# OlegArenz/gmmvi

Measured on AMD Instinct MI355X. Metric: samples_components_per_sec, higher is better.
Workload: dtype f32; 1 GPU; ns: stm target D=20, K=100 components (100/GPU), 100 samples/component, N=10000 samples/iter, SAMTRON (Stein, fixed K, reuse ratio 0, KL trust regions, improvement-based stepsizes); K=100, D=20, N=10000, parallelism=component-shard x1

## Files before the change

gmmvi_amd/_lib.py:

```python
import ctypes as C
import os

_HERE = os.path.dirname(os.path.abspath(__file__))
LIB_PATH = os.environ.get("GMMVI_HIP_LIB", os.path.join(_HERE, "libgmmvi_hip.so"))

GAUSS, STUDENT_T = 0, 1
SELF_NORMALIZED, OWN_SAMPLES_ONLY, EXPLICIT_ESTIMATE = 1, 2, 4
MAX_DIM = 64
MORE_REGISTER_MAX_DIM = 21
MORE_BLOCKED_MIN_DIM, MORE_BLOCKED_MAX_DIM = 64, 128
MAX_DIM_BLOCKED = 512
MAX_DIM_DIAG = 131072
BLOCKED_ABOVE_DEFAULT = 50


_blocked_above = None


def _atoi(text):
    import re
    m = re.match(r"\s*([+-]?\d+)", text)
    return int(m.group(1)) if m else 0


# ... 67 lines not shown
    "gmmvi_target_bnn": (_i, [_p, _i, _i, _i, _i, _p, _p, _u64, _u32, _i, _f, _f, _p, _i, _p, _p]),
    "gmmvi_bnn_predict": (_i, [_p, _i, _i, _i, _p, _i, _p, _i, _p]),
    "gmmvi_target_talos": (_i, [_p, _p, _p, _p, _i, _p, _p]),
    "gmmvi_talos_fk": (_i, [_p, _p, _p, _i, _p, _p]),
    "gmmvi_sample_components": (_i, [_p, _i, _i, _p, _p, _p, _i, _u64, _u64, _i, _p, _p, _p]),
    "gmmvi_philox_normals": (_i, [_p, _u64, _u64, _i, _i, _i, _p]),
    "gmmvi_philox_uniforms": (_i, [_p, _u64, _u64, _i, _i, _p]),
    "gmmvi_stein": (_i, [_p, _i, _i, _p, _p, _i, _p, _p, _p, _p, _p, _i, _i, _p, _p]),
    "gmmvi_more": (_i, [_p, _i, _i, _p, _p, _p, _i, _p, _p, _p, _p, _p, _i, _i, _p, _p, _p]),
    "gmmvi_more_blocked": (_i, [_p, _i, _i, _p, _p, _p, _i, _p, _p, _p, _p, _p, _i, _i, _p, _p, _p]),
    "gmmvi_update_components_kl": (_i, [_p, _i, _i, _p, _p, _p, _p, _p, _f, _f, _p, _p, _p, _p, _p, _p, _p]),
    "gmmvi_update_components_kl_reference": (_i, [_p, _i, _i, _p, _p, _p, _p, _p, _f, _f, _p, _p, _p, _p, _p, _p]),
    "gmmvi_update_components_direct": (_i, [_p, _i, _i, _p, _p, _p, _p, _p, _f, _p, _p, _p]),
    "gmmvi_update_components_iblr": (_i, [_p, _i, _i, _p, _p, _p, _p, _p, _f, _p, _p, _p]),
    "gmmvi_expected_log_ratios": (_i, [_p, _i, _i, _p, _p, _p, _p, _f, _p, _i, _p, _p, _p]),
    "gmmvi_update_weights_kl": (_i, [_p, _i, _p, _p, _p, _f, _p]),
    "gmmvi_update_weights_direct": (_i, [_p, _i, _p, _p, _p, _f]),
    "gmmvi_component_stepsize_improvement": (_i, [_p, _i, _p, _p, _p, _f, _f, _f, _f]),
    "gmmvi_weight_stepsize_improvement": (_i, [_p, _i, _p, _p, _p, _f, _f, _f, _f]),
    "gmmvi_train_iter_samtron": (_i, [_p, _p]),
    "gmmvi_sharded_scratch_floats": (_sz, [_i, _i, _i]),
    "gmmvi_train_iter_sharded_phase": (_i, [_p, _p, _i]),
    "gmmvi_comm_unique_id": (_i, [C.c_char_p]),
    "gmmvi_comm_init": (_i, [_p, C.c_char_p, _i, _i]),
    "gmmvi_comm_destroy": (_i, [_p]),
    "gmmvi_allgather_f32": (_i, [_p, _p, _p, _sz]),
    "gmmvi_allreduce_f32": (_i, [_p, _p, _sz, _i]),
    "gmmvi_combine_partials": (_i, [_p, _i, _i, _i, _p, _p, _p, _p]),
    "gmmvi_diag_packed_stride": (_sz, [_i]),
    "gmmvi_diag_pack": (_i, [_p, _i, _i, _p, _p, _p]),
# ... 41 lines not shown
```

gmmvi_amd/csrc/api.hip:

```cpp
#include "common.h"
#include <cstring>
#include "blocked.h"

std::string g_gmmvi_global_err;

int gmmvi_ws_reserve(gmmvi_ctx* ctx, size_t nbytes) {
    ++ctx->ws_epoch;
    if (nbytes <= ctx->ws_bytes) return GMMVI_OK;
    GMMVI_HIP_CHECK(ctx, hipStreamSynchronize(ctx->stream));
    if (ctx->ws) GMMVI_HIP_CHECK(ctx, hipFree(ctx->ws));
    ctx->ws = nullptr;
    ctx->ws_bytes = 0;
    size_t want = nbytes + nbytes / 2;
    GMMVI_HIP_CHECK(ctx, hipMalloc(&ctx->ws, want));
    ctx->ws_bytes = want;
    return GMMVI_OK;
}

extern "C" {

int gmmvi_device_count(void) {
    int n = 0;
    if (hipGetDeviceCount(&n) != hipSuccess) return 0;
    return n;
// ... 6 lines not shown
    hipError_t e = hipGetDeviceCount(&n);
    if (e != hipSuccess || n == 0)
        return gmmvi_fail(nullptr, GMMVI_ERR_HIP, std::string("no HIP device: ") + hipGetErrorString(e));
    if (device < 0 || device >= n) return gmmvi_fail(nullptr, GMMVI_ERR_ARG, "device index out of range");
    gmmvi_ctx* ctx = new gmmvi_ctx();
    ctx->device = device;
    e = hipSetDevice(device);
    if (e == hipSuccess) e = hipStreamCreateWithFlags(&ctx->stream, hipStreamNonBlocking);
    if (e != hipSuccess) {
        g_gmmvi_global_err = std::string("gmmvi_ctx_create: ") + hipGetErrorString(e);
        delete ctx;
        return GMMVI_ERR_HIP;
    }
    hipDeviceProp_t prop;
    if (hipGetDeviceProperties(&prop, device) == hipSuccess) ctx->num_cus = prop.multiProcessorCount;
    *out = ctx;
    return GMMVI_OK;
}

void gmmvi_ctx_destroy(gmmvi_ctx* ctx) {
    if (!ctx) return;
    gmmvi_comm_destroy(ctx);
    if (ctx->stream) {
        (void)hipStreamSynchronize(ctx->stream);
        (void)hipStreamDestroy(ctx->stream);
    }
    if (ctx->ws) (void)hipFree(ctx->ws);
    if (ctx->arena) (void)hipFree(ctx->arena);
    if (ctx->bimg) (void)hipFree(ctx->bimg);
    if (ctx->up_ring) {
        for (int i = 0; i < gmmvi_ctx::UP_SLOTS; ++i) (void)hipEventDestroy(ctx->up_event[i]);
        (void)hipHostFree(ctx->up_ring);
    }
    if (ctx->defer_ws) (void)hipFree(ctx->defer_ws);
    delete ctx;
}

const char* gmmvi_last_error(gmmvi_ctx* ctx) { return ctx ? ctx->err.c_str() : g_gmmvi_global_err.c_str(); }

int gmmvi_sync(gmmvi_ctx* ctx) {
    GMMVI_HIP_CHECK(ctx, hipStreamSynchronize(ctx->stream));
    return GMMVI_OK;
}

int gmmvi_malloc(gmmvi_ctx* ctx, size_t nbytes, void** out_dev) {
    GMMVI_ARG_CHECK(ctx, out_dev != nullptr);
    *out_dev = nullptr;
    if (nbytes == 0) nbytes = 4;
    GMMVI_HIP_CHECK(ctx, hipSetDevice(ctx->device));
// ... 496 lines not shown
```

gmmvi_amd/csrc/common.h:

```cpp
#pragma once
#include <hip/hip_runtime.h>
#include <cstdio>
#include <cstring>
#include <cstdint>
#include <string>
#include <vector>
#include "../../include/gmmvi_hip.h"
#include "iter_prep.h"

struct CombineJob {
    int R = 0, N = 0, D = 0;
    long part_stride = 0;
    int first_block = 0, blocks = 0;
    const float* lp_parts = nullptr;
    const float* grad_parts = nullptr;
    const float* lp2_parts = nullptr;
    float* lp_out = nullptr;
    float* grad_out = nullptr;
    float* lp2_out = nullptr;
};

struct SampleJob {
    int K = 0, D = 0, uniform_count = 0;
    const float* means = nullptr; const float* chols = nullptr; const int32_t* offsets = nullptr;
// ... 23 lines not shown
    void* arena = nullptr;
    size_t arena_bytes = 0;
    static constexpr int UP_SLOTS = 64;
    static constexpr size_t UP_SLOT_BYTES = 64 * 1024;
    unsigned char* up_ring = nullptr;
    hipEvent_t up_event[UP_SLOTS] = {};
    bool up_used[UP_SLOTS] = {};
    int up_next = 0;
    void* bimg = nullptr;
    size_t bimg_bytes = 0;
    bool defer_combine = false;
    CombineJob pending;
    Riders riders;
    void* defer_ws = nullptr;
    size_t defer_bytes = 0;
    void* comm = nullptr;
    int n_ranks = 1, rank = 0;
    int num_cus = 256;
    unsigned func_attr_done = 0;
    bool prof = false;
    const char* prof_tag = nullptr;
    struct ProfRec { const char* name; hipEvent_t start, stop; double units; };
    std::vector<ProfRec> prof_recs;
};

struct GmmviProfScope {
    gmmvi_ctx* ctx; hipEvent_t stop = nullptr;
    GmmviProfScope(gmmvi_ctx* c, const char* name, double units = 0.0) : ctx(c) {
        if (!c->prof) return;
        hipEvent_t start;
// ... 48 lines not shown
CombineJob gmmvi_take_pending_combine(gmmvi_ctx* ctx, int threads, int first_block, bool light = false);
Riders gmmvi_take_pending_riders(gmmvi_ctx* ctx, int first_block, int threads, bool prep_only = false);
int gmmvi_flush_pending_riders(gmmvi_ctx* ctx);
struct SteinSlab;
int gmmvi_stein_partials(gmmvi_ctx* ctx, int K, int D, const float* packed_dev, const float* X_dev, int N, const float* ld_dev,
                         const float* qgrad_dev, const float* bg_dev, const float* tgrad_dev, int flags, SteinSlab* slab);
int gmmvi_stein_finalize_slab(gmmvi_ctx* ctx, int K, int D, const SteinSlab& slab, int N, int flags, const float* packed_dev,
                              float* H_neg_out_dev, float* g_neg_out_dev);
int gmmvi_update_components_kl_from_slab(gmmvi_ctx* ctx, int K, int D, const SteinSlab& slab, int N, int stein_flags,
                                         const float* packed_old_dev, float* H_neg_dev, float* g_neg_dev, float* means_dev,
                                         float* chols_dev, const float* stepsizes_dev, float temperature, float l2_init,
                                         float* last_eta_dev, float* l2_dev, float* num_received_updates_dev,
                                         int32_t* success_out_dev, float* packed_out_dev);
int gmmvi_update_weights_internal(gmmvi_ctx* ctx, int mode, int K, float* logw_dev, const float* E_dev,
                                  const float* stepsize_dev, float beta, float* kl_eta_out_dev, float* exp_out_dev);

inline int gmmvi_padded_dim(int D) {
    static const int dps[] = {2, 4, 8, 10, 12, 16, 20, 24, 32, 40, 50, 64};
    for (int dp : dps) if (D <= dp) return dp;
    return -1;
}

#define GMMVI_DISPATCH_DP(DPVAL, ...)                  \
    switch (DPVAL) {                                   \
        case 2:  { constexpr int DP = 2;  __VA_ARGS__; } break;  \
        case 4:  { constexpr int DP = 4;  __VA_ARGS__; } break;  \
        case 8:  { constexpr int DP = 8;  __VA_ARGS__; } break;  \
        case 10: { constexpr int DP = 10; __VA_ARGS__; } break;  \
        case 12: { constexpr int DP = 12; __VA_ARGS__; } break;  \
        case 16: { constexpr int DP = 16; __VA_ARGS__; } break;  \
// ... 103 lines not shown
```

gmmvi_amd/csrc/fused.hip:

```cpp
#include "common.h"
#include "stepsize_rules.h"
#include "iter_prep.h"
#include "stein_finalize.h"

namespace {
struct Arena {
    float *ld, *lq, *qgrad, *bg, *H, *g, *E;
    int32_t *mapping, *success;
};

}

static int arena_reserve(gmmvi_ctx* ctx, size_t floats) {
    if (floats * sizeof(float) <= ctx->arena_bytes) return GMMVI_OK;
    GMMVI_HIP_CHECK(ctx, hipStreamSynchronize(ctx->stream));
    if (ctx->arena) GMMVI_HIP_CHECK(ctx, hipFree(ctx->arena));
    ctx->arena = nullptr;
    ctx->arena_bytes = 0;
    size_t want = floats * sizeof(float) * 3 / 2;
    GMMVI_HIP_CHECK(ctx, hipMalloc(&ctx->arena, want));
    ctx->arena_bytes = want;
    return GMMVI_OK;
}

// ... 2 lines not shown
        int rc__ = (call);             \
        if (rc__ != GMMVI_OK) return rc__; \
    } while (0)

static int train_iter_samtron_body(gmmvi_ctx* ctx, const gmmvi_samtron_plan* p);

extern "C" int gmmvi_train_iter_samtron(gmmvi_ctx* ctx, const gmmvi_samtron_plan* p) {
    GMMVI_ARG_CHECK(ctx, ctx != nullptr);
    int rc = gmmvi_flush_pending_combine(ctx);
    if (rc == GMMVI_OK) rc = train_iter_samtron_body(ctx, p);
    if (rc != GMMVI_OK) {
        ctx->pending = CombineJob();
        ctx->riders.prep_blocks = ctx->riders.sample_blocks = 0;
        ctx->defer_combine = false;
        ctx->prof_tag = nullptr;
    }
    return rc;
}

static int train_iter_samtron_body(gmmvi_ctx* ctx, const gmmvi_samtron_plan* p) {
    GMMVI_ARG_CHECK(ctx, p != nullptr);
    GMMVI_ARG_CHECK(ctx, (p->target_kind >= 0 && p->target_kind <= 2) || p->target_kind == 4);
    GMMVI_ARG_CHECK(ctx, p->target_kind != 2 || (p->logreg_A && p->logreg_M >= 1 && p->logreg_prior_std > 0.f));
    GMMVI_ARG_CHECK(ctx, p->target_kind != 4 || (p->talos_model && p->talos_context && p->D == 34));
    const int K = p->K, D = p->D, N = p->N;
    GMMVI_ARG_CHECK(ctx, K >= 1 && D >= 1 && D < GMMVI_MAX_DIM && N >= 1);
    GMMVI_ARG_CHECK(ctx, p->means && p->chols && p->logw && p->packed && p->packed_new && p->stepsizes && p->last_eta &&
                             p->l2 && p->num_updates && p->offsets && p->bg_logw && p->db_samples && p->db_tlp &&
                             p->db_tgrad && p->db_mapping && p->reward_next && p->wstate);
    GMMVI_ARG_CHECK(ctx, p->n_old >= 0 && p->max_per_component >= 0 && p->phase >= 0 && p->phase <= 2);
// ... 103 lines not shown
    ctx->defer_combine = true;
    ctx->prof_tag = "sweep_post";
    int rc_post = gmmvi_mixture_eval(ctx, GMMVI_GAUSS, 0.f, K, D, p->packed_new, p->logw, xa, Na, a.ld, a.lq, nullptr);
    ctx->defer_combine = false;
    ctx->prof_tag = nullptr;
    GMMVI_TRY(rc_post);
    if (p->presample_next && n_old == 0) {
        const int max_pc = p->max_per_component > 0 ? p->max_per_component : (N + K - 1) / K;
        SampleJob& sj = ctx->riders.sample;
        sj.K = K; sj.D = D; sj.uniform_count = (long)K * max_pc == N ? max_pc : 0;
        sj.means = p->means; sj.chols = p->chols; sj.offsets = p->offsets;
        sj.seed = p->seed; sj.first_index = p->first_index + (uint64_t)N;
        sj.X = x + (size_t)N * D; sj.mapping = p->db_mapping + N; sj.mapping_base = p->mapping_base + K;
        ctx->riders.sample_blocks = K * ((max_pc + 255) / 256);
    }
    GMMVI_TRY(gmmvi_expected_log_ratios(ctx, K, Na, a.ld, a.bg, tlp_a, a.lq, p->temperature, p->logw,
                                        (p->stein_flags & GMMVI_SELF_NORMALIZED) ? 1 : 0, a.E, p->reward_next, nullptr));
    GMMVI_TRY(gmmvi_flush_pending_riders(ctx));
    if (K > 1) {
        GMMVI_TRY(gmmvi_update_weights_internal(ctx, p->weight_update_mode == 0 ? 0 : 1, K, p->logw, a.E, p->wstate,
                                                p->temperature, nullptr, p->weight_slot));
    }
    return GMMVI_OK;
}


namespace {
struct ShardArena { float *ld, *lq, *bg, *qgrad, *H, *g, *E; int32_t* success; };
}
extern "C" size_t gmmvi_sharded_scratch_floats(int K, int D, int N) {
    if (K < 1 || D < 1 || N < 1) return 0;
    return (size_t)K * N + 2 * (size_t)N + (size_t)N * D + (size_t)K * D * D + (size_t)K * D + 2 * (size_t)K + 64;
}
static void shard_arena(float* base, int K, int D, int N, ShardArena& a) {
    a.ld = base; base += (size_t)K * N;
    a.lq = base; base += N;
    a.bg = base; base += N;
// ... 141 lines not shown
```

gmmvi_amd/csrc/weights.hip:

```cpp
#include "common.h"
#include "riders.h"
#include "stepsize_rules.h"
#include "wave_reduce.h"
#include "combine.h"
#include <cfloat>

namespace {

__device__ __forceinline__ float wsum(float v) { return gmmvi_wave_sum(v); }
__device__ __forceinline__ float wmax(float v) { return gmmvi_wave_max(v); }

__device__ float block_max(float v, float* red) {
    v = wmax(v);
    __syncthreads();
    if ((threadIdx.x & 63) == 0) red[threadIdx.x >> 6] = v;
    __syncthreads();
    return fmaxf(fmaxf(red[0], red[1]), fmaxf(red[2], red[3]));
}
__device__ float block_sum(float v, float* red) {
    v = wsum(v);
    __syncthreads();
    if ((threadIdx.x & 63) == 0) red[threadIdx.x >> 6] = v;
    __syncthreads();
    return (red[0] + red[1]) + (red[2] + red[3]);
}

template <int R>
__device__ __forceinline__ void elr_accumulate(int N, const float* __restrict__ row, const float* __restrict__ bg,
                                               const float* __restrict__ tlp, const float* __restrict__ logq, int Rrt, float beta,
                                               float& m, float& s, float& se, float& s2) {
    constexpr int B = 4;
    for (int n0 = threadIdx.x; n0 < N; n0 += 1024 * B) {
        float av[B], rv[B];
#pragma unroll
        for (int u = 0; u < B; ++u) {
            const int n = min(n0 + 1024 * u, N - 1);
            av[u] = row[n] - bg[n];
            float lq;
            if constexpr (R == 0) lq = logq[n];
            else if constexpr (R > 0) lq = combine_log_values_n<R>(logq, N, n);
            else lq = combine_log_values(logq, Rrt, N, n);
            rv[u] = tlp[n] - beta * lq;
        }
#pragma unroll
        for (int u = 0; u < B; ++u) {
            if (n0 + 1024 * u < N) {
                const float a = av[u], rho = rv[u];
                const float mn = fmaxf(m, a);
                const float sc = __expf(m - mn), e = __expf(a - mn);
                s = fmaf(s, sc, e);
                se = fmaf(se, sc, e * rho);
                s2 = fmaf(s2, sc * sc, e * e);
                m = mn;
            }
        }
    }
}

__device__ __forceinline__ void elr_body(int N, const float* __restrict__ ld, const float* __restrict__ bg,
                                         const float* __restrict__ tlp, const float* __restrict__ logq, int logq_R,
                                         float beta, const float* __restrict__ logw, int self_normalized,
                                         float* __restrict__ E_out, float* __restrict__ reward_out,
                                         float* __restrict__ ess_out) {
    __shared__ float red[4][16];
    const int k = blockIdx.x;
    const float* row = ld + (size_t)k * N;
    float m = -3.0e38f, s = 0.f, se = 0.f, s2 = 0.f;
    switch (logq_R) {
        case 0: elr_accumulate<0>(N, row, bg, tlp, logq, 0, beta, m, s, se, s2); break;
        case 2: elr_accumulate<2>(N, row, bg, tlp, logq, 2, beta, m, s, se, s2); break;
        case 3: elr_accumulate<3>(N, row, bg, tlp, logq, 3, beta, m, s, se, s2); break;
        case 4: elr_accumulate<4>(N, row, bg, tlp, logq, 4, beta, m, s, se, s2); break;
        case 5: elr_accumulate<5>(N, row, bg, tlp, logq, 5, beta, m, s, se, s2); break;
        case 6: elr_accumulate<6>(N, row, bg, tlp, logq, 6, beta, m, s, se, s2); break;
        case 7: elr_accumulate<7>(N, row, bg, tlp, logq, 7, beta, m, s, se, s2); break;
        case 8: elr_accumulate<8>(N, row, bg, tlp, logq, 8, beta, m, s, se, s2); break;
        case 10: elr_accumulate<10>(N, row, bg, tlp, logq, 10, beta, m, s, se, s2); break;
        case 12: elr_accumulate<12>(N, row, bg, tlp, logq, 12, beta, m, s, se, s2); break;
        case 16: elr_accumulate<16>(N, row, bg, tlp, logq, 16, beta, m, s, se, s2); break;
        default: elr_accumulate<-1>(N, row, bg, tlp, logq, logq_R, beta, m, s, se, s2); break;
    }
    const float mw = wmax(m);
    const float f = __expf(m - mw);
    s = wsum(s * f); se = wsum(se * f); s2 = wsum(s2 * f * f);
    const int lane = threadIdx.x & 63, wave = threadIdx.x >> 6;
    if (lane == 0) { red[0][wave] = mw; red[1][wave] = s; red[2][wave] = se; red[3][wave] = s2; }
    __syncthreads();
    if (threadIdx.x == 0) {
        float M = -3.0e38f;
        for (int w = 0; w < 16; ++w) M = fmaxf(M, red[0][w]);
        float S = 0.f, SE = 0.f, S2 = 0.f;
        for (int w = 0; w < 16; ++w) {
            const float g = __expf(red[0][w] - M);
            S = fmaf(red[1][w], g, S); SE = fmaf(red[2][w], g, SE); S2 = fmaf(red[3][w], g * g, S2);
        }
        const float E = self_normalized ? SE / S : SE * __expf(M) / (float)N;
        if (E_out) E_out[k] = E;
        if (reward_out) reward_out[k] = beta * logw[k] + E;
        if (ess_out) ess_out[k] = (S * S) / S2;
    }
}

__global__ __launch_bounds__(1024) void elr_kernel(int N, const float* __restrict__ ld, const float* __restrict__ bg,
                                                   const float* __restrict__ tlp, const float* __restrict__ logq, int logq_R,
                                                   float beta, const float* __restrict__ logw, int self_normalized,
                                                   float* __restrict__ E_out, float* __restrict__ reward_out,
                                                   float* __restrict__ ess_out) {
    elr_body(N, ld, bg, tlp, logq, logq_R, beta, logw, self_normalized, E_out, reward_out, ess_out);
}

template <int DP>
__global__ __launch_bounds__(1024) void elr_riders_kernel(int N, const float* __restrict__ ld, const float* __restrict__ bg,
                                                          const float* __restrict__ tlp, const float* __restrict__ logq,
                                                          int logq_R, float beta, const float* __restrict__ logw,
                                                          int self_normalized, float* __restrict__ E_out,
                                                          float* __restrict__ reward_out, float* __restrict__ ess_out,
                                                          Riders riders) {
    extern __shared__ __align__(16) float sm_riders[];
    if (riders_carried<DP>(riders, sm_riders)) return;
    elr_body(N, ld, bg, tlp, logq, logq_R, beta, logw, self_normalized, E_out, reward_out, ess_out);
}

__device__ float wave_lse(const float* v, int K) {
    const int t = threadIdx.x;
    float m = -3.0e38f;
    for (int i = t; i < K; i += 64) m = fmaxf(m, v[i]);
    m = wmax(m);
    float s = 0.f;
    for (int i = t; i < K; i += 64) s += __expf(v[i] - m);
    s = wsum(s);
    return m + __logf(s);
}

__device__ float weights_kl(float eta, float beta, const float* lw, const float* E, float* nl, int K) {
    const int t = threadIdx.x;
// ... 73 lines not shown
    }
    if (lb == ub) {
    } else if (ub_ok) {
        eta = expf(ub);
        kl = weights_kl_reg<NE>(eta, beta, lw, E, h, v);
    } else {
        updated = false;
        kl = -1.f; eta = -1.f;
    }
#pragma unroll
    for (int e = 0; e < NE; ++e)
        if (h[e]) nl[t + 64 * e] = v[e];
    __syncthreads();
}

__global__ __launch_bounds__(64) void update_weights_kernel(int mode, int K, float* __restrict__ logw,
                                                            const float* __restrict__ E_in, const float* __restrict__ stepsize,
                                                            float beta, float* __restrict__ kl_eta_out,
                                                            float* __restrict__ exp_out) {
    extern __shared__ float sm[];
    float* lw = sm; float* E = sm + K; float* nl = sm + 2 * K;
    const int t = threadIdx.x;
    for (int i = t; i < K; i += 64) { lw[i] = logw[i]; E[i] = E_in[i]; nl[i] = logw[i]; }
    __syncthreads();
    if (K <= 1) return;
    const float bound = stepsize[0];
    float kl = -1.f, eta = -1.f;
    bool updated = true;
    if (mode == 1) {
        for (int i = t; i < K; i += 64) nl[i] = lw[i] + bound / beta * E[i];
        __syncthreads();
        float l = wave_lse(nl, K);
        for (int i = t; i < K; i += 64) nl[i] = fmaxf(nl[i] - l, -69.07f);
        __syncthreads();
        l = wave_lse(nl, K);
// ... 31 lines not shown
        }
    }
    if (!updated) {
        for (int i = t; i < K; i += 64) nl[i] = lw[i];
        __syncthreads();
    }
    const float l = wave_lse(nl, K);
    for (int i = t; i < K; i += 64) {
        const float v = nl[i] - l;
        logw[i] = v;
        if (exp_out) exp_out[i] = expf(v);
    }
    if (t == 0 && kl_eta_out) { kl_eta_out[0] = kl; kl_eta_out[1] = eta; }
}

__global__ void component_stepsize_kernel(int K, float* __restrict__ stepsizes, const float* __restrict__ prev,
                                          const float* __restrict__ last, float mn, float mx, float inc, float dec) {
    const int k = blockIdx.x * blockDim.x + threadIdx.x;
    if (k >= K) return;
    stepsizes[k] = component_stepsize_rule(stepsizes[k], prev[k], last[k], mn, mx, inc, dec);
}

__global__ __launch_bounds__(64) void weight_stepsize_kernel(int K, const float* __restrict__ logw,
                                                             const float* __restrict__ rewards_last, float* __restrict__ state,
                                                             float mn, float mx, float inc, float dec) {
    weight_stepsize_wave(K, logw, rewards_last, state, mn, mx, inc, dec, threadIdx.x);
}

}

extern "C" {

int gmmvi_expected_log_ratios(gmmvi_ctx* ctx, int K, int N, const float* ld_dev, const float* bg_dev,
                              const float* tlp_dev, const float* logq_dev, float beta, const float* logw_dev,
                              int self_normalized, float* E_out_dev, float* reward_out_dev, float* ess_out_dev) {
    GMMVI_ARG_CHECK(ctx, K >= 1 && N >= 1);
    GMMVI_ARG_CHECK(ctx, ld_dev && bg_dev && tlp_dev && logq_dev && logw_dev);
    int logq_R = 0;
    {
        const CombineJob& j = ctx->pending;
        if (j.R > 0 && j.lp_out == logq_dev && j.N == N && !j.grad_out && !j.lp2_out) {
            logq_R = j.R;
            logq_dev = j.lp_parts;
            ctx->pending = CombineJob();
        } else {
            int rc = gmmvi_flush_pending_combine(ctx);
            if (rc != GMMVI_OK) return rc;
        }
    }
    GMMVI_PROF(ctx, "expected_log_ratios");
    const Riders riders = gmmvi_take_pending_riders(ctx, K, 1024);
    if (riders.prep_blocks + riders.sample_blocks > 0) {
        const int dp = gmmvi_padded_dim(riders.sample_blocks > 0 ? riders.sample.D : 2);
        GMMVI_DISPATCH_DP(dp, hipLaunchKernelGGL((elr_riders_kernel<DP>), dim3(K + riders.prep_blocks + riders.sample_blocks),
                                                 dim3(1024), riders_lds_bytes(riders), ctx->stream, N, ld_dev, bg_dev, tlp_dev,
                                                 logq_dev, logq_R, beta, logw_dev, self_normalized, E_out_dev, reward_out_dev,
                                                 ess_out_dev, riders));
    } else {
        hipLaunchKernelGGL(elr_kernel, dim3(K), dim3(1024), 0, ctx->stream, N, ld_dev, bg_dev, tlp_dev, logq_dev, logq_R, beta,
                           logw_dev, self_normalized, E_out_dev, reward_out_dev, ess_out_dev);
    }
    GMMVI_LAUNCH_CHECK(ctx);
    return GMMVI_OK;
}

}

int gmmvi_update_weights_internal(gmmvi_ctx* ctx, int mode, int K, float* logw_dev, const float* E_dev,
                                  const float* stepsize_dev, float beta, float* kl_eta_out_dev, float* exp_out_dev) {
    GMMVI_ARG_CHECK(ctx, K >= 1 && K <= 4096);
    GMMVI_ARG_CHECK(ctx, logw_dev && E_dev && stepsize_dev);
    GMMVI_PROF(ctx, "update_weights");
    hipLaunchKernelGGL(update_weights_kernel, dim3(1), dim3(64), (size_t)3 * K * sizeof(float), ctx->stream, mode, K,
                       logw_dev, E_dev, stepsize_dev, beta, kl_eta_out_dev, exp_out_dev);
    GMMVI_LAUNCH_CHECK(ctx);
    return GMMVI_OK;
}

extern "C" {

int gmmvi_update_weights_kl(gmmvi_ctx* ctx, int K, float* logw_dev, const float* E_dev, const float* stepsize_dev,
                            float beta, float* kl_eta_out_dev) {
    return gmmvi_update_weights_internal(ctx, 0, K, logw_dev, E_dev, stepsize_dev, beta, kl_eta_out_dev, nullptr);
}

int gmmvi_update_weights_direct(gmmvi_ctx* ctx, int K, float* logw_dev, const float* E_dev,
                                const float* stepsize_dev, float beta) {
    return gmmvi_update_weights_internal(ctx, 1, K, logw_dev, E_dev, stepsize_dev, beta, nullptr, nullptr);
}

int gmmvi_component_stepsize_improvement(gmmvi_ctx* ctx, int K, float* stepsizes_dev, const float* rewards_prev_dev,
                                         const float* rewards_last_dev, float min_stepsize, float max_stepsize,
                                         float inc_factor, float dec_factor) {
// ... 21 lines not shown
```

gmmvi_amd/hip_ops.py:

```python
import math

import numpy as np

from . import _lib
from .device import DeviceArray

F32, I32 = np.dtype(np.float32), np.dtype(np.int32)


def _req(a, shape, dtype=F32, name="array"):
    if not isinstance(a, DeviceArray):
        raise TypeError(f"{name}: expected DeviceArray, got {type(a)}")
    if a.dtype != dtype or tuple(a.shape) != tuple(shape):
        raise ValueError(f"{name}: expected {dtype}{tuple(shape)}, got {a.dtype}{a.shape}")
    return a.ptr


def _opt(a, shape, dtype=F32, name="array"):
    return None if a is None else _req(a, shape, dtype, name)


def packed_stride(d):
    s = int(_lib.load().gmmvi_packed_stride(int(d)))
    if s == 0:
# ... 411 lines not shown
def expected_log_ratios(ctx, ld, bg, tlp, logq, beta, logw, self_normalized=True, reward_out=None, want_ess=False):
    k, n = ld.shape
    _req(ld, (k, n), name="ld"); _req(bg, (n,), name="bg"); _req(tlp, (n,), name="tlp"); _req(logq, (n,), name="logq")
    _req(logw, (k,), name="logw")
    if reward_out is not None:
        _req(reward_out, (k,), name="reward_out")
    e = ctx.empty((k,))
    ess = ctx.empty((k,)) if want_ess else None
    ctx.check(ctx.lib.gmmvi_expected_log_ratios(ctx.handle, k, n, ld.ptr, bg.ptr, tlp.ptr, logq.ptr, float(beta),
                                                logw.ptr, 1 if self_normalized else 0, e.ptr,
                                                None if reward_out is None else reward_out.ptr,
                                                None if ess is None else ess.ptr))
    return e, ess


def update_weights(ctx, mode, logw, e, stepsize, beta, want_info=False):
    k = logw.shape[0]
    _req(logw, (k,), name="logw"); _req(e, (k,), name="E"); _req(stepsize, (1,), name="stepsize")
    info = ctx.empty((2,)) if (want_info and mode == "trust-region") else None
    if mode == "trust-region":
        ctx.check(ctx.lib.gmmvi_update_weights_kl(ctx.handle, k, logw.ptr, e.ptr, stepsize.ptr, float(beta),
                                                  None if info is None else info.ptr))
    else:
        ctx.check(ctx.lib.gmmvi_update_weights_direct(ctx.handle, k, logw.ptr, e.ptr, stepsize.ptr, float(beta)))
    return info


def component_stepsize_improvement(ctx, stepsizes, prev, last, mn, mx, inc, dec):
    k = stepsizes.shape[0]
    _req(stepsizes, (k,), name="stepsizes"); _req(prev, (k,), name="prev"); _req(last, (k,), name="last")
# ... 111 lines not shown
```

include/gmmvi_hip.h:

```cpp
#ifndef GMMVI_HIP_H
#define GMMVI_HIP_H

#include <stddef.h>
#include <stdint.h>

#ifdef __cplusplus
extern "C" {
#endif

typedef struct gmmvi_ctx gmmvi_ctx;

enum gmmvi_status {
    GMMVI_OK = 0,
    GMMVI_ERR_HIP = -1,
    GMMVI_ERR_ARG = -2,
    GMMVI_ERR_RCCL = -3,
    GMMVI_ERR_STATE = -4
};

enum gmmvi_family {
    GMMVI_GAUSS = 0,
    GMMVI_STUDENT_T = 1
};

// ... 121 lines not shown
                                         float temperature, float l2_init, float* last_eta_dev, float* l2_dev,
                                         float* num_received_updates_dev, int32_t* success_out_dev, float* kl_out_dev,
                                         int32_t* n_probes_out_dev);
int gmmvi_update_components_direct(gmmvi_ctx* ctx, int K, int D, float* means_dev, float* chols_dev,
                                   const float* H_neg_dev, const float* g_neg_dev, const float* stepsizes_dev,
                                   float l2_init, float* l2_dev, float* num_received_updates_dev,
                                   int32_t* success_out_dev);
int gmmvi_update_components_iblr(gmmvi_ctx* ctx, int K, int D, float* means_dev, float* chols_dev,
                                 const float* H_neg_dev, const float* g_neg_dev, const float* stepsizes_dev,
                                 float l2_init, float* l2_dev, float* num_received_updates_dev,
                                 int32_t* success_out_dev);

int gmmvi_expected_log_ratios(gmmvi_ctx* ctx, int K, int N, const float* ld_dev, const float* bg_dev,
                              const float* tlp_dev, const float* logq_dev, float beta, const float* logw_dev,
                              int self_normalized, float* E_out_dev, float* reward_out_dev, float* ess_out_dev);
int gmmvi_update_weights_kl(gmmvi_ctx* ctx, int K, float* logw_dev, const float* E_dev, const float* stepsize_dev,
                            float beta, float* kl_eta_out_dev);
int gmmvi_update_weights_direct(gmmvi_ctx* ctx, int K, float* logw_dev, const float* E_dev,
                                const float* stepsize_dev, float beta);
int gmmvi_component_stepsize_improvement(gmmvi_ctx* ctx, int K, float* stepsizes_dev, const float* rewards_prev_dev,
                                         const float* rewards_last_dev, float min_stepsize, float max_stepsize,
                                         float inc_factor, float dec_factor);
int gmmvi_weight_stepsize_improvement(gmmvi_ctx* ctx, int K, const float* logw_dev, const float* rewards_last_dev,
                                      float* state_dev, float min_stepsize, float max_stepsize, float inc_factor,
                                      float dec_factor);

typedef struct gmmvi_samtron_plan {
    int32_t K, D, N;
    int32_t target_kind;
    int32_t target_family, target_K;
// ... 125 lines not shown
```

Baseline: 5.026 billion samples*components/s.

## Fuse weight update into expected-log-ratio kernel and split samples across blocks

Splits each component's expected-log-ratio reduction over several blocks, sized by CU count and capped at 8, and merges the partial log-sum-exp stats with an atomic-ticket last-block pattern. The block that finishes last then runs the weight update in one wave, so the separate update_weights kernel launch is no longer needed. This targets launch overhead and the poor occupancy of having only K blocks for K=100. In exchange it adds device-wide tickets and fences, persistent ticket state that has to be reset on errors, and a larger shared-memory footprint.

```diff
diff --git a/gmmvi_amd/_lib.py b/gmmvi_amd/_lib.py
--- a/gmmvi_amd/_lib.py
+++ b/gmmvi_amd/_lib.py
@@ -105,6 +105,7 @@
     "gmmvi_update_components_direct": (_i, [_p, _i, _i, _p, _p, _p, _p, _p, _f, _p, _p, _p]),
     "gmmvi_update_components_iblr": (_i, [_p, _i, _i, _p, _p, _p, _p, _p, _f, _p, _p, _p]),
     "gmmvi_expected_log_ratios": (_i, [_p, _i, _i, _p, _p, _p, _p, _f, _p, _i, _p, _p, _p]),
+    "gmmvi_expected_log_ratios_update_weights": (_i, [_p, _i, _i, _p, _p, _p, _p, _f, _p, _i, _p, _p, _p, _i, _p, _p, _p]),
     "gmmvi_update_weights_kl": (_i, [_p, _i, _p, _p, _p, _f, _p]),
     "gmmvi_update_weights_direct": (_i, [_p, _i, _p, _p, _p, _f]),
     "gmmvi_component_stepsize_improvement": (_i, [_p, _i, _p, _p, _p, _f, _f, _f, _f]),
diff --git a/gmmvi_amd/csrc/api.hip b/gmmvi_amd/csrc/api.hip
--- a/gmmvi_amd/csrc/api.hip
+++ b/gmmvi_amd/csrc/api.hip
@@ -44,6 +44,16 @@
     }
     hipDeviceProp_t prop;
     if (hipGetDeviceProperties(&prop, device) == hipSuccess) ctx->num_cus = prop.multiProcessorCount;
+    const size_t elr_bytes = gmmvi_ctx::ELR_TICKET_WORDS * sizeof(int32_t) + (size_t)gmmvi_ctx::ELR_MAX_BLOCKS * 4 * sizeof(float);
+    e = hipMalloc(&ctx->elr_state, elr_bytes);
+    if (e == hipSuccess) e = hipMemsetAsync(ctx->elr_state, 0, elr_bytes, ctx->stream);
+    if (e != hipSuccess) {
+        g_gmmvi_global_err = std::string("gmmvi_ctx_create: ") + hipGetErrorString(e);
+        if (ctx->elr_state) (void)hipFree(ctx->elr_state);
+        (void)hipStreamDestroy(ctx->stream);
+        delete ctx;
+        return GMMVI_ERR_HIP;
+    }
     *out = ctx;
     return GMMVI_OK;
 }
@@ -63,6 +73,7 @@
         (void)hipHostFree(ctx->up_ring);
     }
     if (ctx->defer_ws) (void)hipFree(ctx->defer_ws);
+    if (ctx->elr_state) (void)hipFree(ctx->elr_state);
     delete ctx;
 }
 
diff --git a/gmmvi_amd/csrc/common.h b/gmmvi_amd/csrc/common.h
--- a/gmmvi_amd/csrc/common.h
+++ b/gmmvi_amd/csrc/common.h
@@ -61,6 +61,8 @@
     Riders riders;
     void* defer_ws = nullptr;
     size_t defer_bytes = 0;
+    static constexpr int ELR_TICKET_WORDS = 1024, ELR_MAX_BLOCKS = 1024;
+    void* elr_state = nullptr;
     void* comm = nullptr;
     int n_ranks = 1, rank = 0;
     int num_cus = 256;
@@ -139,6 +141,7 @@
                                          int32_t* success_out_dev, float* packed_out_dev);
 int gmmvi_update_weights_internal(gmmvi_ctx* ctx, int mode, int K, float* logw_dev, const float* E_dev,
                                   const float* stepsize_dev, float beta, float* kl_eta_out_dev, float* exp_out_dev);
+int gmmvi_elr_reset_tickets(gmmvi_ctx* ctx);
 
 inline int gmmvi_padded_dim(int D) {
     static const int dps[] = {2, 4, 8, 10, 12, 16, 20, 24, 32, 40, 50, 64};
diff --git a/gmmvi_amd/csrc/fused.hip b/gmmvi_amd/csrc/fused.hip
--- a/gmmvi_amd/csrc/fused.hip
+++ b/gmmvi_amd/csrc/fused.hip
@@ -40,6 +40,9 @@
         ctx->riders.prep_blocks = ctx->riders.sample_blocks = 0;
         ctx->defer_combine = false;
         ctx->prof_tag = nullptr;
+        const std::string err = ctx->err;
+        (void)gmmvi_elr_reset_tickets(ctx);
+        ctx->err = err;
     }
     return rc;
 }
@@ -173,13 +176,11 @@
         sj.X = x + (size_t)N * D; sj.mapping = p->db_mapping + N; sj.mapping_base = p->mapping_base + K;
         ctx->riders.sample_blocks = K * ((max_pc + 255) / 256);
     }
-    GMMVI_TRY(gmmvi_expected_log_ratios(ctx, K, Na, a.ld, a.bg, tlp_a, a.lq, p->temperature, p->logw,
-                                        (p->stein_flags & GMMVI_SELF_NORMALIZED) ? 1 : 0, a.E, p->reward_next, nullptr));
+    GMMVI_TRY(gmmvi_expected_log_ratios_update_weights(ctx, K, Na, a.ld, a.bg, tlp_a, a.lq, p->temperature, p->logw,
+                                                       (p->stein_flags & GMMVI_SELF_NORMALIZED) ? 1 : 0, a.E, p->reward_next,
+                                                       nullptr, p->weight_update_mode == 0 ? 0 : 1, p->wstate, nullptr,
+                                                       p->weight_slot));
     GMMVI_TRY(gmmvi_flush_pending_riders(ctx));
-    if (K > 1) {
-        GMMVI_TRY(gmmvi_update_weights_internal(ctx, p->weight_update_mode == 0 ? 0 : 1, K, p->logw, a.E, p->wstate,
-                                                p->temperature, nullptr, p->weight_slot));
-    }
     return GMMVI_OK;
 }
 
diff --git a/gmmvi_amd/csrc/weights.hip b/gmmvi_amd/csrc/weights.hip
--- a/gmmvi_amd/csrc/weights.hip
+++ b/gmmvi_amd/csrc/weights.hip
@@ -26,15 +26,16 @@
 }
 
 template <int R>
-__device__ __forceinline__ void elr_accumulate(int N, const float* __restrict__ row, const float* __restrict__ bg,
-                                               const float* __restrict__ tlp, const float* __restrict__ logq, int Rrt, float beta,
+__device__ __forceinline__ void elr_accumulate(int n_begin, int n_end, int N, const float* __restrict__ row,
+                                               const float* __restrict__ bg, const float* __restrict__ tlp,
+                                               const float* __restrict__ logq, int Rrt, float beta,
                                                float& m, float& s, float& se, float& s2) {
     constexpr int B = 4;
-    for (int n0 = threadIdx.x; n0 < N; n0 += 1024 * B) {
+    for (int n0 = n_begin + threadIdx.x; n0 < n_end; n0 += 1024 * B) {
         float av[B], rv[B];
 #pragma unroll
         for (int u = 0; u < B; ++u) {
-            const int n = min(n0 + 1024 * u, N - 1);
+            const int n = min(n0 + 1024 * u, n_end - 1);
             av[u] = row[n] - bg[n];
             float lq;
             if constexpr (R == 0) lq = logq[n];
@@ -44,7 +45,7 @@
         }
 #pragma unroll
         for (int u = 0; u < B; ++u) {
-            if (n0 + 1024 * u < N) {
+            if (n0 + 1024 * u < n_end) {
                 const float a = av[u], rho = rv[u];
                 const float mn = fmaxf(m, a);
                 const float sc = __expf(m - mn), e = __expf(a - mn);
@@ -57,28 +58,46 @@
     }
 }
 
-__device__ __forceinline__ void elr_body(int N, const float* __restrict__ ld, const float* __restrict__ bg,
+__device__ __forceinline__ void agent_release() {
+    __builtin_amdgcn_fence(__ATOMIC_RELEASE, "agent");
+    asm volatile("s_waitcnt vmcnt(0)" ::: "memory");
+}
+__device__ __forceinline__ void agent_acquire() { __builtin_amdgcn_fence(__ATOMIC_ACQUIRE, "agent"); }
+__device__ __forceinline__ int ticket_draw(int* t) { return __hip_atomic_fetch_add(t, 1, __ATOMIC_RELAXED, __HIP_MEMORY_SCOPE_AGENT); }
+__device__ __forceinline__ void ticket_reset(int* t) { __hip_atomic_store(t, 0, __ATOMIC_RELAXED, __HIP_MEMORY_SCOPE_AGENT); }
+__device__ __forceinline__ void agent_store(float* p, float v) { __hip_atomic_store(p, v, __ATOMIC_RELAXED, __HIP_MEMORY_SCOPE_AGENT); }
+__device__ __forceinline__ float agent_load(const float* p) { return __hip_atomic_load(p, __ATOMIC_RELAXED, __HIP_MEMORY_SCOPE_AGENT); }
+
+struct ElrRanges { int S, L; float* parts; int* tickets; };
+struct ElrTail { int mode; float* logw; const float* stepsize; float* kl_eta_out; float* exp_out; int* ticket; };
+
+__device__ __forceinline__ void update_weights_wave(float* sm, int mode, int K, float* __restrict__ logw,
+                                                    const float* __restrict__ E_in, const float* __restrict__ stepsize,
+                                                    float beta, float* __restrict__ kl_eta_out, float* __restrict__ exp_out);
+
+__device__ __forceinline__ void elr_body(int K, int N, const float* __restrict__ ld, const float* __restrict__ bg,
                                          const float* __restrict__ tlp, const float* __restrict__ logq, int logq_R,
-                                         float beta, const float* __restrict__ logw, int self_normalized,
-                                         float* __restrict__ E_out, float* __restrict__ reward_out,
-                                         float* __restrict__ ess_out) {
-    __shared__ float red[4][16];
-    const int k = blockIdx.x;
+                                         float beta, const float* logw, int self_normalized, float* E_out,
+                                         float* __restrict__ reward_out, float* __restrict__ ess_out, const ElrRanges& rg,
+                                         const ElrTail& tail, float* sm) {
+    __shared__ float red[5][16];
+    const int k = (int)blockIdx.x / rg.S, r = (int)blockIdx.x - k * rg.S;
+    const int nb = r * rg.L, ne = min(N, nb + rg.L);
     const float* row = ld + (size_t)k * N;
     float m = -3.0e38f, s = 0.f, se = 0.f, s2 = 0.f;
     switch (logq_R) {
-        case 0: elr_accumulate<0>(N, row, bg, tlp, logq, 0, beta, m, s, se, s2); break;
-        case 2: elr_accumulate<2>(N, row, bg, tlp, logq, 2, beta, m, s, se, s2); break;
-        case 3: elr_accumulate<3>(N, row, bg, tlp, logq, 3, beta, m, s, se, s2); break;
-        case 4: elr_accumulate<4>(N, row, bg, tlp, logq, 4, beta, m, s, se, s2); break;
-        case 5: elr_accumulate<5>(N, row, bg, tlp, logq, 5, beta, m, s, se, s2); break;
-        case 6: elr_accumulate<6>(N, row, bg, tlp, logq, 6, beta, m, s, se, s2); break;
-        case 7: elr_accumulate<7>(N, row, bg, tlp, logq, 7, beta, m, s, se, s2); break;
-        case 8: elr_accumulate<8>(N, row, bg, tlp, logq, 8, beta, m, s, se, s2); break;
-        case 10: elr_accumulate<10>(N, row, bg, tlp, logq, 10, beta, m, s, se, s2); break;
-        case 12: elr_accumulate<12>(N, row, bg, tlp, logq, 12, beta, m, s, se, s2); break;
-        case 16: elr_accumulate<16>(N, row, bg, tlp, logq, 16, beta, m, s, se, s2); break;
-        default: elr_accumulate<-1>(N, row, bg, tlp, logq, logq_R, beta, m, s, se, s2); break;
+        case 0: elr_accumulate<0>(nb, ne, N, row, bg, tlp, logq, 0, beta, m, s, se, s2); break;
+        case 2: elr_accumulate<2>(nb, ne, N, row, bg, tlp, logq, 2, beta, m, s, se, s2); break;
+        case 3: elr_accumulate<3>(nb, ne, N, row, bg, tlp, logq, 3, beta, m, s, se, s2); break;
+        case 4: elr_accumulate<4>(nb, ne, N, row, bg, tlp, logq, 4, beta, m, s, se, s2); break;
+        case 5: elr_accumulate<5>(nb, ne, N, row, bg, tlp, logq, 5, beta, m, s, se, s2); break;
+        case 6: elr_accumulate<6>(nb, ne, N, row, bg, tlp, logq, 6, beta, m, s, se, s2); break;
+        case 7: elr_accumulate<7>(nb, ne, N, row, bg, tlp, logq, 7, beta, m, s, se, s2); break;
+        case 8: elr_accumulate<8>(nb, ne, N, row, bg, tlp, logq, 8, beta, m, s, se, s2); break;
+        case 10: elr_accumulate<10>(nb, ne, N, row, bg, tlp, logq, 10, beta, m, s, se, s2); break;
+        case 12: elr_accumulate<12>(nb, ne, N, row, bg, tlp, logq, 12, beta, m, s, se, s2); break;
+        case 16: elr_accumulate<16>(nb, ne, N, row, bg, tlp, logq, 16, beta, m, s, se, s2); break;
+        default: elr_accumulate<-1>(nb, ne, N, row, bg, tlp, logq, logq_R, beta, m, s, se, s2); break;
     }
     const float mw = wmax(m);
     const float f = __expf(m - mw);
@@ -94,31 +113,66 @@
             const float g = __expf(red[0][w] - M);
             S = fmaf(red[1][w], g, S); SE = fmaf(red[2][w], g, SE); S2 = fmaf(red[3][w], g * g, S2);
         }
-        const float E = self_normalized ? SE / S : SE * __expf(M) / (float)N;
-        if (E_out) E_out[k] = E;
-        if (reward_out) reward_out[k] = beta * logw[k] + E;
-        if (ess_out) ess_out[k] = (S * S) / S2;
-    }
-}
-
-__global__ __launch_bounds__(1024) void elr_kernel(int N, const float* __restrict__ ld, const float* __restrict__ bg,
+        bool complete = true;
+        if (rg.S > 1) {
+            float* mine = rg.parts + 4 * (size_t)blockIdx.x;
+            agent_store(mine, M); agent_store(mine + 1, S); agent_store(mine + 2, SE); agent_store(mine + 3, S2);
+            agent_release();
+            complete = ticket_draw(rg.tickets + k) == rg.S - 1;
+            if (complete) {
+                ticket_reset(rg.tickets + k);
+                agent_acquire();
+                const float* part = rg.parts + 4 * (size_t)k * rg.S;
+                M = -3.0e38f;
+                for (int i = 0; i < rg.S; ++i) M = fmaxf(M, agent_load(part + 4 * i));
+                S = 0.f; SE = 0.f; S2 = 0.f;
+                for (int i = 0; i < rg.S; ++i) {
+                    const float g = __expf(agent_load(part + 4 * i) - M);
+                    S = fmaf(agent_load(part + 4 * i + 1), g, S);
+                    SE = fmaf(agent_load(part + 4 * i + 2), g, SE);
+                    S2 = fmaf(agent_load(part + 4 * i + 3), g * g, S2);
+                }
+            }
+        }
+        bool last = false;
+        if (complete) {
+            const float E = self_normalized ? SE / S : SE * __expf(M) / (float)N;
+            if (E_out) E_out[k] = E;
+            if (reward_out) reward_out[k] = beta * logw[k] + E;
+            if (ess_out) ess_out[k] = (S * S) / S2;
+            if (tail.mode >= 0) {
+                agent_release();
+                last = ticket_draw(tail.ticket) == K - 1;
+                if (last) ticket_reset(tail.ticket);
+            }
+        }
+        red[4][0] = last ? 1.f : 0.f;
+    }
+    if (tail.mode < 0) return;
+    __syncthreads();
+    if (red[4][0] == 0.f || threadIdx.x >= 64) return;
+    agent_acquire();
+    update_weights_wave(sm, tail.mode, K, tail.logw, E_out, tail.stepsize, beta, tail.kl_eta_out, tail.exp_out);
+}
+
+__global__ __launch_bounds__(1024) void elr_kernel(int K, int N, const float* __restrict__ ld, const float* __restrict__ bg,
                                                    const float* __restrict__ tlp, const float* __restrict__ logq, int logq_R,
-                                                   float beta, const float* __restrict__ logw, int self_normalized,
-                                                   float* __restrict__ E_out, float* __restrict__ reward_out,
-                                                   float* __restrict__ ess_out) {
-    elr_body(N, ld, bg, tlp, logq, logq_R, beta, logw, self_normalized, E_out, reward_out, ess_out);
+                                                   float beta, const float* logw, int self_normalized, float* E_out,
+                                                   float* __restrict__ reward_out, float* __restrict__ ess_out,
+                                                   ElrRanges rg, ElrTail tail) {
+    extern __shared__ __align__(16) float sm_elr[];
+    elr_body(K, N, ld, bg, tlp, logq, logq_R, beta, logw, self_normalized, E_out, reward_out, ess_out, rg, tail, sm_elr);
 }
 
 template <int DP>
-__global__ __launch_bounds__(1024) void elr_riders_kernel(int N, const float* __restrict__ ld, const float* __restrict__ bg,
+__global__ __launch_bounds__(1024) void elr_riders_kernel(int K, int N, const float* __restrict__ ld, const float* __restrict__ bg,
                                                           const float* __restrict__ tlp, const float* __restrict__ logq,
-                                                          int logq_R, float beta, const float* __restrict__ logw,
-                                                          int self_normalized, float* __restrict__ E_out,
-                                                          float* __restrict__ reward_out, float* __restrict__ ess_out,
-                                                          Riders riders) {
+                                                          int logq_R, float beta, const float* logw, int self_normalized,
+                                                          float* E_out, float* __restrict__ reward_out,
+                                                          float* __restrict__ ess_out, ElrRanges rg, ElrTail tail, Riders riders) {
     extern __shared__ __align__(16) float sm_riders[];
     if (riders_carried<DP>(riders, sm_riders)) return;
-    elr_body(N, ld, bg, tlp, logq, logq_R, beta, logw, self_normalized, E_out, reward_out, ess_out);
+    elr_body(K, N, ld, bg, tlp, logq, logq_R, beta, logw, self_normalized, E_out, reward_out, ess_out, rg, tail, sm_riders);
 }
 
 __device__ float wave_lse(const float* v, int K) {
@@ -222,11 +276,9 @@
     __syncthreads();
 }
 
-__global__ __launch_bounds__(64) void update_weights_kernel(int mode, int K, float* __restrict__ logw,
-                                                            const float* __restrict__ E_in, const float* __restrict__ stepsize,
-                                                            float beta, float* __restrict__ kl_eta_out,
-                                                            float* __restrict__ exp_out) {
-    extern __shared__ float sm[];
+__device__ __forceinline__ void update_weights_wave(float* sm, int mode, int K, float* __restrict__ logw,
+                                                    const float* __restrict__ E_in, const float* __restrict__ stepsize,
+                                                    float beta, float* __restrict__ kl_eta_out, float* __restrict__ exp_out) {
     float* lw = sm; float* E = sm + K; float* nl = sm + 2 * K;
     const int t = threadIdx.x;
     for (int i = t; i < K; i += 64) { lw[i] = logw[i]; E[i] = E_in[i]; nl[i] = logw[i]; }
@@ -288,6 +340,14 @@
     if (t == 0 && kl_eta_out) { kl_eta_out[0] = kl; kl_eta_out[1] = eta; }
 }
 
+__global__ __launch_bounds__(64) void update_weights_kernel(int mode, int K, float* __restrict__ logw,
+                                                            const float* __restrict__ E_in, const float* __restrict__ stepsize,
+                                                            float beta, float* __restrict__ kl_eta_out,
+                                                            float* __restrict__ exp_out) {
+    extern __shared__ float sm[];
+    update_weights_wave(sm, mode, K, logw, E_in, stepsize, beta, kl_eta_out, exp_out);
+}
+
 __global__ void component_stepsize_kernel(int K, float* __restrict__ stepsizes, const float* __restrict__ prev,
                                           const float* __restrict__ last, float mn, float mx, float inc, float dec) {
     const int k = blockIdx.x * blockDim.x + threadIdx.x;
@@ -303,13 +363,19 @@
 
 }
 
-extern "C" {
-
-int gmmvi_expected_log_ratios(gmmvi_ctx* ctx, int K, int N, const float* ld_dev, const float* bg_dev,
-                              const float* tlp_dev, const float* logq_dev, float beta, const float* logw_dev,
-                              int self_normalized, float* E_out_dev, float* reward_out_dev, float* ess_out_dev) {
-    GMMVI_ARG_CHECK(ctx, K >= 1 && N >= 1);
-    GMMVI_ARG_CHECK(ctx, ld_dev && bg_dev && tlp_dev && logq_dev && logw_dev);
+static void elr_ranges(const gmmvi_ctx* ctx, int K, int N, int& S, int& L) {
+    int s = ctx->num_cus / K;
+    if (s > 8) s = 8;
+    if (s < 1 || (long)K * s > gmmvi_ctx::ELR_MAX_BLOCKS || K + 1 > gmmvi_ctx::ELR_TICKET_WORDS) s = 1;
+    const long l = (((long)N + s - 1) / s + 1023) / 1024 * 1024;
+    S = (int)((N + l - 1) / l);
+    L = S > 1 ? (int)l : N;
+}
+
+static int elr_launch(gmmvi_ctx* ctx, int K, int N, const float* ld_dev, const float* bg_dev, const float* tlp_dev,
+                      const float* logq_dev, float beta, const float* logw_dev, int self_normalized, float* E_out_dev,
+                      float* reward_out_dev, float* ess_out_dev, int tail_mode, float* logw_rw_dev, const float* stepsize_dev,
+                      float* kl_eta_out_dev, float* exp_out_dev) {
     int logq_R = 0;
     {
         const CombineJob& j = ctx->pending;
@@ -322,22 +388,41 @@
             if (rc != GMMVI_OK) return rc;
         }
     }
+    int* tickets = (int*)ctx->elr_state;
+    ElrRanges rg{1, N, (float*)(tickets + gmmvi_ctx::ELR_TICKET_WORDS), tickets + 1};
+    elr_ranges(ctx, K, N, rg.S, rg.L);
+    const ElrTail tail{tail_mode, logw_rw_dev, stepsize_dev, kl_eta_out_dev, exp_out_dev, tickets};
+    const size_t tail_lds = tail_mode >= 0 ? (size_t)3 * K * sizeof(float) : 0;
     GMMVI_PROF(ctx, "expected_log_ratios");
-    const Riders riders = gmmvi_take_pending_riders(ctx, K, 1024);
+    const int own = K * rg.S;
+    const Riders riders = gmmvi_take_pending_riders(ctx, own, 1024);
     if (riders.prep_blocks + riders.sample_blocks > 0) {
         const int dp = gmmvi_padded_dim(riders.sample_blocks > 0 ? riders.sample.D : 2);
-        GMMVI_DISPATCH_DP(dp, hipLaunchKernelGGL((elr_riders_kernel<DP>), dim3(K + riders.prep_blocks + riders.sample_blocks),
-                                                 dim3(1024), riders_lds_bytes(riders), ctx->stream, N, ld_dev, bg_dev, tlp_dev,
-                                                 logq_dev, logq_R, beta, logw_dev, self_normalized, E_out_dev, reward_out_dev,
-                                                 ess_out_dev, riders));
+        const size_t lds = riders_lds_bytes(riders) > tail_lds ? riders_lds_bytes(riders) : tail_lds;
+        GMMVI_DISPATCH_DP(dp, hipLaunchKernelGGL((elr_riders_kernel<DP>), dim3(own + riders.prep_blocks + riders.sample_blocks),
+                                                 dim3(1024), lds, ctx->stream, K, N, ld_dev, bg_dev, tlp_dev, logq_dev, logq_R,
+                                                 beta, logw_dev, self_normalized, E_out_dev, reward_out_dev, ess_out_dev, rg, tail,
+                                                 riders));
     } else {
-        hipLaunchKernelGGL(elr_kernel, dim3(K), dim3(1024), 0, ctx->stream, N, ld_dev, bg_dev, tlp_dev, logq_dev, logq_R, beta,
-                           logw_dev, self_normalized, E_out_dev, reward_out_dev, ess_out_dev);
+        hipLaunchKernelGGL(elr_kernel, dim3(own), dim3(1024), tail_lds, ctx->stream, K, N, ld_dev, bg_dev, tlp_dev, logq_dev,
+                           logq_R, beta, logw_dev, self_normalized, E_out_dev, reward_out_dev, ess_out_dev, rg, tail);
     }
     GMMVI_LAUNCH_CHECK(ctx);
     return GMMVI_OK;
 }
 
+int gmmvi_elr_reset_tickets(gmmvi_ctx* ctx) {
+    GMMVI_HIP_CHECK(ctx, hipMemsetAsync(ctx->elr_state, 0, gmmvi_ctx::ELR_TICKET_WORDS * sizeof(int32_t), ctx->stream));
+    return GMMVI_OK;
+}
+
+extern "C" int gmmvi_expected_log_ratios(gmmvi_ctx* ctx, int K, int N, const float* ld_dev, const float* bg_dev,
+                                         const float* tlp_dev, const float* logq_dev, float beta, const float* logw_dev,
+                                         int self_normalized, float* E_out_dev, float* reward_out_dev, float* ess_out_dev) {
+    GMMVI_ARG_CHECK(ctx, K >= 1 && N >= 1);
+    GMMVI_ARG_CHECK(ctx, ld_dev && bg_dev && tlp_dev && logq_dev && logw_dev);
+    return elr_launch(ctx, K, N, ld_dev, bg_dev, tlp_dev, logq_dev, beta, logw_dev, self_normalized, E_out_dev, reward_out_dev,
+                      ess_out_dev, -1, nullptr, nullptr, nullptr, nullptr);
 }
 
 int gmmvi_update_weights_internal(gmmvi_ctx* ctx, int mode, int K, float* logw_dev, const float* E_dev,
@@ -351,6 +436,29 @@
     return GMMVI_OK;
 }
 
+extern "C" int gmmvi_expected_log_ratios_update_weights(gmmvi_ctx* ctx, int K, int N, const float* ld_dev, const float* bg_dev,
+                                                        const float* tlp_dev, const float* logq_dev, float beta,
+                                                        float* logw_dev, int self_normalized, float* E_out_dev,
+                                                        float* reward_out_dev, float* ess_out_dev, int mode,
+                                                        const float* stepsize_dev, float* kl_eta_out_dev, float* exp_out_dev) {
+    GMMVI_ARG_CHECK(ctx, K >= 1 && N >= 1 && (mode == 0 || mode == 1));
+    GMMVI_ARG_CHECK(ctx, ld_dev && bg_dev && tlp_dev && logq_dev && logw_dev && E_out_dev && stepsize_dev);
+    const bool tail = K > 1 && K <= 4096;
+    int rc = elr_launch(ctx, K, N, ld_dev, bg_dev, tlp_dev, logq_dev, beta, logw_dev, self_normalized, E_out_dev, reward_out_dev,
+                        ess_out_dev, tail ? mode : -1, logw_dev, stepsize_dev, kl_eta_out_dev, exp_out_dev);
+    if (K > 1 && !tail) {
+        if (rc == GMMVI_OK) rc = gmmvi_flush_pending_riders(ctx);
+        if (rc == GMMVI_OK)
+            rc = gmmvi_update_weights_internal(ctx, mode, K, logw_dev, E_out_dev, stepsize_dev, beta, kl_eta_out_dev, exp_out_dev);
+    }
+    if (rc != GMMVI_OK) {
+        const std::string err = ctx->err;
+        (void)gmmvi_elr_reset_tickets(ctx);
+        ctx->err = err;
+    }
+    return rc;
+}
+
 extern "C" {
 
 int gmmvi_update_weights_kl(gmmvi_ctx* ctx, int K, float* logw_dev, const float* E_dev, const float* stepsize_dev,
diff --git a/gmmvi_amd/hip_ops.py b/gmmvi_amd/hip_ops.py
--- a/gmmvi_amd/hip_ops.py
+++ b/gmmvi_amd/hip_ops.py
@@ -449,6 +449,26 @@
     return e, ess
 
 
+def expected_log_ratios_update_weights(ctx, mode, ld, bg, tlp, logq, beta, logw, stepsize, self_normalized=True,
+                                       reward_out=None, want_ess=False, want_info=False, exp_out=None):
+    k, n = ld.shape
+    _req(ld, (k, n), name="ld"); _req(bg, (n,), name="bg"); _req(tlp, (n,), name="tlp"); _req(logq, (n,), name="logq")
+    _req(logw, (k,), name="logw"); _req(stepsize, (1,), name="stepsize")
+    if reward_out is not None:
+        _req(reward_out, (k,), name="reward_out")
+    if exp_out is not None:
+        _req(exp_out, (k,), name="exp_out")
+    e = ctx.empty((k,))
+    ess = ctx.empty((k,)) if want_ess else None
+    info = ctx.empty((2,)) if (want_info and mode == "trust-region") else None
+    ctx.check(ctx.lib.gmmvi_expected_log_ratios_update_weights(
+        ctx.handle, k, n, ld.ptr, bg.ptr, tlp.ptr, logq.ptr, float(beta), logw.ptr, 1 if self_normalized else 0, e.ptr,
+        None if reward_out is None else reward_out.ptr, None if ess is None else ess.ptr,
+        0 if mode == "trust-region" else 1, stepsize.ptr, None if info is None else info.ptr,
+        None if exp_out is None else exp_out.ptr))
+    return e, ess, info
+
+
 def update_weights(ctx, mode, logw, e, stepsize, beta, want_info=False):
     k = logw.shape[0]
     _req(logw, (k,), name="logw"); _req(e, (k,), name="E"); _req(stepsize, (1,), name="stepsize")
diff --git a/include/gmmvi_hip.h b/include/gmmvi_hip.h
--- a/include/gmmvi_hip.h
+++ b/include/gmmvi_hip.h
@@ -159,6 +159,10 @@
 int gmmvi_expected_log_ratios(gmmvi_ctx* ctx, int K, int N, const float* ld_dev, const float* bg_dev,
                               const float* tlp_dev, const float* logq_dev, float beta, const float* logw_dev,
                               int self_normalized, float* E_out_dev, float* reward_out_dev, float* ess_out_dev);
+int gmmvi_expected_log_ratios_update_weights(gmmvi_ctx* ctx, int K, int N, const float* ld_dev, const float* bg_dev,
+                                             const float* tlp_dev, const float* logq_dev, float beta, float* logw_dev,
+                                             int self_normalized, float* E_out_dev, float* reward_out_dev, float* ess_out_dev,
+                                             int mode, const float* stepsize_dev, float* kl_eta_out_dev, float* exp_out_dev);
 int gmmvi_update_weights_kl(gmmvi_ctx* ctx, int K, float* logw_dev, const float* E_dev, const float* stepsize_dev,
                             float beta, float* kl_eta_out_dev);
 int gmmvi_update_weights_direct(gmmvi_ctx* ctx, int K, float* logw_dev, const float* E_dev,
```

Result: slower. 4.636 billion samples*components/s (-7.8%).
